# alibaba/euler

Measured on NVIDIA H100. Metric: sampled_edges_per_sec, higher is better.
Workload: dtype u64 ids / f32 weights+features (f64 CDF compare)

## Files before the change

### euler_b200/_lib.py

```python
import ctypes as C
import os

_HERE = os.path.dirname(os.path.abspath(__file__))
SO_PATH = os.path.join(_HERE, "lib", "libeuler_b200.so")

EU_RNG_MINSTD = 0
EU_RNG_PHILOX = 1


class EulerError(RuntimeError):
    pass


class GraphDesc(C.Structure):
    _fields_ = [
        ("n_nodes", C.c_int64), ("n_edge_types", C.c_int32), ("n_node_types", C.c_int32),
        ("ids", C.c_void_p), ("node_type", C.c_void_p), ("node_w", C.c_void_p),
        ("grp_ptr", C.c_void_p), ("nbr", C.c_void_p), ("cum_w", C.c_void_p), ("grp_cum", C.c_void_p),
        ("w", C.c_void_p), ("feat_dim", C.c_int32), ("feat", C.c_void_p),
        ("sampler_order", C.c_void_p), ("n_feat_slots", C.c_int32), ("feat_slot_dims", C.c_void_p),
        ("n_u64_slots", C.c_int32), ("u64_ptr", C.c_void_p), ("u64_val", C.c_void_p),
        ("n_bin_slots", C.c_int32), ("bin_ptr", C.c_void_p), ("bin_val", C.c_void_p),
    ]

# ... 69 lines not shown
    "eu_graph_feat_dim": (_I32, [_P]),
    "eu_graph_hbm_bytes": (_I64, [_P]),
    "eu_graph_export": (C.c_int, [_P] * 9),
    "eu_graph_edge_type_id": (_I32, [_P, C.c_char_p]),
    "eu_graph_node_type_id": (_I32, [_P, C.c_char_p]),
    "eu_graph_dense_feature_id": (_I32, [_P, C.c_char_p]),
    "eu_graph_dense_feature_dim": (_I32, [_P, _I32]),
    "eu_graph_sparse_feature_id": (_I32, [_P, C.c_char_p]),
    "eu_graph_binary_feature_id": (_I32, [_P, C.c_char_p]),
    "eu_get_sparse_feature": (C.c_int, [_P, _P, _I64, _I32, _I64, _I64, _P, _P]),
    "eu_get_sparse_feature_host": (C.c_int, [_P, _P, _I64, _I32, _I64, _I64, _P, _P, _P]),
    "eu_get_binary_feature": (C.c_int, [_P, _P, _I64, _I32, _I64, _P, _P]),
    "eu_get_binary_feature_host": (C.c_int, [_P, _P, _I64, _I32, _I64, _P, _P, _P]),
    "eu_ctx_create": (C.c_int, [_P, C.c_int, _U64, _P, C.POINTER(_P)]),
    "eu_ctx_destroy": (C.c_int, [_P]),
    "eu_ctx_set_stream": (C.c_int, [_P, _P]),
    "eu_ctx_seed": (C.c_int, [_P, _U64]),
    "eu_ctx_set_engines": (C.c_int, [_P, _I32, _P]),
    "eu_ctx_reserve": (C.c_int, [_P, _I64]),
    "eu_ctx_sync": (C.c_int, [_P]),
    "eu_ctx_draws": (C.c_int, [_P, C.POINTER(_U64)]),
    "eu_ctx_profile": (C.c_int, [_P, C.c_int]),
    "eu_ctx_profile_read": (C.c_int, [_P, C.c_char_p, _I64]),
    "eu_sample_neighbor": (C.c_int, [_P, _P, _I64, _P, _I32, _I32, _I64, _P, _P, _P]),
    "eu_sample_neighbor_host": (C.c_int, [_P, _P, _I64, _P, _I32, _I32, _I64, _P, _P, _P]),
    "eu_sample_neighbor_raw": (C.c_int, [_P, _P, _I64, _P, _I32, _I32, _P, _P, _P]),
    "eu_sample_neighbor_raw_host": (C.c_int, [_P, _P, _I64, _P, _I32, _I32, _P, _P, _P]),
    "eu_get_sorted_full_neighbor": (C.c_int, [_P, _P, _I64, _P, _I32, _I64, _P, _P, _P, _P]),
    "eu_get_top_k_neighbor": (C.c_int, [_P, _P, _I64, _P, _I32, _I32, _I64, _P, _P, _P]),
    "eu_sample_neighbor_layerwise": (C.c_int, [_P, _P, _I64, _I32, _P, _I32, _I32, _I64, _I32, _P, _P]),
    "eu_sparse_get_adj": (C.c_int, [_P, _P, _P, _I64, _I32, _I32, _P, _I32, _P]),
    "eu_sparse_get_adj_coo": (C.c_int, [_P, _P, _P, _I64, _I32, _I32, _P, _I32, _I64, _P, _P, _P]),
    "eu_gen_pair_count": (_I64, [_I32, _I32, _I32]),
    "eu_gen_pair": (C.c_int, [_P, _P, _I64, _I32, _I32, _I32, _P]),
    "eu_sample_fanout": (C.c_int, [_P, _P, _I64, _P, _I32, _P, _I32, _I64, _P, _P, _P]),
    "eu_sample_fanout_batched": (C.c_int, [_P, _P, _I32, _I64, _P, _I32, _P, _I32, _I64, _P, _P, _P]),
    "eu_sample_fanout_host": (C.c_int, [_P, _P, _I64, _P, _I32, _P, _I32, _I64, _P, _P, _P]),
    "eu_sample_fanout_batched_host": (C.c_int, [_P, _P, _I32, _I64, _P, _I32, _P, _I32, _I64, _P, _P, _P]),
    "eu_sample_fanout_with_feature": (C.c_int, [_P, _P, _I64, _P, _I32, _P, _I32, _I64, _P, _P, _P, _P, _I32, _P, _P, _P, _I32, _P, _P,
                                                _P, _P]),
    "eu_sage_mean_aggregate_host": (C.c_int, [_P, _P, _I64, _I32, _I32, _P]),
    "eu_sample_node": (C.c_int, [_P, _I32, _P, _I32, _P]),
    "eu_sample_node_host": (C.c_int, [_P, _I32, _P, _I32, _P]),
    "eu_build_alias_table": (C.c_int, [_P, _I64, _P, _P, _P]),
    "eu_graph_load_inspect": (C.c_int, [C.c_char_p, C.c_int, C.c_int, _P, _P, _P, _P, _I64, _P, _P]),
    "eu_random_walk": (C.c_int, [_P, _P, _I64, _P, _I32, _I32, _F, _F, _I64, _P]),
# ... 97 lines not shown
```

### euler_b200/csrc/capi.cu

```cuda
#include <stdio.h>
#include <stdlib.h>
#include <string.h>

#include <algorithm>
#include <map>
#include <mutex>
#include <string>

#include "internal.h"

namespace eu {

__global__ void k_seed(EuRngState* rs, int n, unsigned long long seed0, const unsigned long long* seeds) {
  const int e = blockIdx.x * blockDim.x + threadIdx.x;
  if (e >= n) return;
  const unsigned long long seed = seeds ? seeds[e] : seed0 + (unsigned long long)e;
  EuRngState* r = rs + e;
  unsigned long long x = seed % 2147483647ull;
  r->x = x == 0 ? 1u : (uint32_t)x;
  r->x_prev = r->x;
  r->draws = 0;
  r->calls = 0;
  r->blocks_done = 0;
  r->key = seed * 0x9E3779B97F4A7C15ull;
// ... 25 lines not shown
  int rc;
  if ((table_slots > c->tab_set_slots || rows > c->cap_rows) && (rc = refuse_growth_in_capture(c, "the sampling scratch"))) return rc;
  if (table_slots > c->tab_set_slots) {
    EU_CUDA(cudaStreamSynchronize(c->stream));
    const int64_t slots = table_slots + 64;
    if ((rc = regrow(&c->d_dedup, 2 * slots))) return rc;
    c->tab_set_slots = slots;
    for (int64_t off = 0; off < 2 * slots; off += (int64_t)1 << 20) {
      int64_t n = std::min<int64_t>((int64_t)1 << 20, 2 * slots - off);
      EU_CUDA(cudaMemset2DAsync(&c->d_dedup[off].key, sizeof(HashSlot), 0x00, 8, (size_t)n, c->stream));
      EU_CUDA(cudaMemset2DAsync(&c->d_dedup[off].row, sizeof(HashSlot), 0xFF, 8, (size_t)n, c->stream));
    }
  }
  if (rows <= c->cap_rows) return EU_OK;
  EU_CUDA(cudaStreamSynchronize(c->stream));
  if ((rc = regrow(&c->d_first, rows))) return rc;
  if ((rc = regrow(&c->d_rowof, rows))) return rc;
  if ((rc = regrow(&c->d_elig, rows))) return rc;
  if ((rc = regrow(&c->d_state, rows))) return rc;
  if ((rc = regrow(&c->d_emask, rows / 32 + 2))) return rc;
  if ((rc = regrow(&c->d_woff, rows / 32 + 2))) return rc;
  if ((rc = regrow(&c->d_blkpre, rows / 256 + 66))) return rc;
  if ((rc = regrow(&c->d_blkmul, rows / 256 + 66))) return rc;
  if ((rc = regrow(&c->d_live, rows))) return rc;
  if ((rc = regrow(&c->d_dup, rows))) return rc;
  if (!c->d_nlive && (rc = regrow(&c->d_nlive, 4))) return rc;
  if ((rc = regrow(&c->d_front[0], rows))) return rc;
  if ((rc = regrow(&c->d_front[1], rows))) return rc;
  c->cap_rows = rows;
  return EU_OK;
}

int ctx_misc(eu_ctx* c, int64_t bytes) {
  if (bytes <= c->misc_bytes) return EU_OK;
  if (int rc0 = refuse_growth_in_capture(c, "the op scratch")) return rc0;
  EU_CUDA(cudaStreamSynchronize(c->stream));
  char* p = (char*)c->d_misc;
  int rc = regrow(&p, bytes);
  c->d_misc = p;
  if (rc) { c->misc_bytes = 0; return rc; }
  c->misc_bytes = bytes;
  return EU_OK;
}

int agg_reserve(eu_ctx* c, int64_t rows, int64_t table_slots) {
  if (rows <= c->agg_rows && table_slots <= c->agg_slots) return EU_OK;
  int rc;
// ... 201 lines not shown
```

### euler_b200/csrc/internal.h

```cpp
#pragma once
#include <cuda_runtime.h>
#include <stdint.h>

#include <atomic>
#include <string>
#include <vector>

#include "../../include/euler_b200.h"
#include "common.cuh"

namespace eu {

void set_error(const char* fmt, ...);
extern std::atomic<uint64_t> g_launches;

#define EU_CUDA(call)                                                                    \
  do {                                                                                   \
    cudaError_t _e = (call);                                                             \
    if (_e != cudaSuccess) {                                                             \
      ::eu::set_error("%s:%d %s -> %s", __FILE__, __LINE__, #call, cudaGetErrorString(_e)); \
      return EU_ERR_CUDA;                                                                \
    }                                                                                    \
  } while (0)

// ... 80 lines not shown
};

struct eu_ctx {
  eu_graph* g = nullptr;
  eu_rng_kind rng = EU_RNG_MINSTD;
  uint64_t seed = 0;
  cudaStream_t stream = nullptr;
  EuRngState* d_rng = nullptr;
  int n_eng = 1;
  int64_t cap_rows = 0;
  eu::HashSlot* d_dedup = nullptr;
  int64_t tab_set_slots = 0;
  int32_t* d_first = nullptr;
  int64_t* d_rowof = nullptr;
  uint8_t* d_elig = nullptr;
  uint32_t* d_state = nullptr;
  uint32_t* d_emask = nullptr;
  uint32_t* d_woff = nullptr;
  uint32_t* d_blkpre = nullptr;
  uint32_t* d_blkmul = nullptr;
  int32_t* d_live = nullptr;
  int32_t* d_dup = nullptr;
  unsigned int* d_nlive = nullptr;
  unsigned long long* d_front[2] = {nullptr, nullptr};
  int64_t agg_rows = 0, agg_slots = 0;
  unsigned long long* d_agg_tab = nullptr;
  int32_t* d_agg_src = nullptr;
  int32_t* d_agg_rep = nullptr;
  uint32_t* d_agg_slot = nullptr;
  unsigned int* d_agg_nrep = nullptr;
  void* d_misc = nullptr;
  int64_t misc_bytes = 0;
  float* d_walkv = nullptr;
  long long walkv_cap = 0;
  cudaStream_t aux[2] = {nullptr, nullptr};
  cudaEvent_t ev_fork = nullptr, ev_join[2] = {nullptr, nullptr};
  void* h_pin = nullptr;
  int64_t pin_bytes = 0;
  void* d_stage = nullptr;
  int64_t stage_bytes = 0;
  bool prof = false;
  struct ProfRec { const char* name; int64_t rows; cudaEvent_t e0, e1; };
  std::vector<ProfRec> prof_recs;
};

struct EuProfScope {
// ... 43 lines not shown
```

### euler_b200/csrc/sample.cu

```cuda
#include <algorithm>

#include <stdlib.h>

#include "internal.h"

namespace eu {

struct ETypes {
  int32_t K;
  int32_t v[EU_MAX_ETYPES];
};

struct Geom {
  int32_t nb;
  int32_t nblk_b;
  int64_t rows_b;
  int64_t rows_pad;
  int64_t cap_b;
  const int32_t* rows_act;
};

__global__ void k_dedup_insert(HashSlot* tabs, Geom gm, const unsigned long long* __restrict__ seeds) {
  const int b = blockIdx.y;
  const int64_t li = blockIdx.x * (int64_t)blockDim.x + threadIdx.x;
// ... 35 lines not shown
  if (mode == 1) {
    float s = 0.f;
    for (int32_t i = 0; i < et.K; ++i) {
      int32_t t = et.v[i];
      if (t < 0 || t >= T) return false;
      float pre = t > 0 ? grp_cum_at(g, row, t - 1) : 0.f;
      s = __fadd_rn(s, __fsub_rn(grp_cum_at(g, row, t), pre));
    }
    return s != 0.f;
  }
  return grp_cum_at(g, row, T - 1) != 0.f;
}

struct PrepOut {
  unsigned long long* eng_ids;
  long long* out_ids;
  float* out_w;
  int32_t* out_t;
  int32_t count;
  long long default_node;
  HashSlot* next_tabs;
  int64_t next_cap_b;
  int32_t* live;
  unsigned int* n_live;
  int32_t* dup;
  unsigned int* n_dup;
};

static constexpr int kPrepBlock = 256;

__global__ void __launch_bounds__(kPrepBlock) k_prepare(DevGraph g, const HashSlot* tabs, Geom gm,
                                                        const unsigned long long* __restrict__ seeds,
                                                        ETypes et, int mode, uint32_t F, unsigned long long draws_per_row,
                                                        int32_t* first, int64_t* rowof, uint32_t* emask, uint32_t* wmul,
                                                        uint32_t* blkpre, uint32_t* blkmul, EuRngState* rngs, PrepOut po) {
  __shared__ uint32_t s_w[kPrepBlock / 32];
  __shared__ uint32_t s_l[kPrepBlock / 32];
  __shared__ uint32_t s_d[kPrepBlock / 32];
  __shared__ uint32_t s_z[kPrepBlock / 32];
  __shared__ bool s_last;
  const int b = blockIdx.y;
  const int64_t li = blockIdx.x * (int64_t)kPrepBlock + threadIdx.x;
  const int64_t ii = b * gm.rows_pad + li;
  const int lane = threadIdx.x & 31, wid = threadIdx.x >> 5;
  EuRngState* rng = rngs + b;
  bool e = false;
  bool own = false;
  bool dflt = false;
  const int64_t rows_here = gm.rows_act ? (int64_t)gm.rows_act[b] : gm.rows_b;
  const uint32_t nblk_act = (uint32_t)max((int64_t)1, (rows_here + kPrepBlock - 1) / kPrepBlock);
  if (blockIdx.x >= nblk_act) return;
  if (li < rows_here) {
    const int64_t w = b * gm.rows_b + li;
    const unsigned long long id = seeds[w];
    const int64_t f = tabs ? dedup_first(tabs + (int64_t)b * (gm.cap_b + 1), (unsigned long long)dedup_cap_eff(gm.cap_b, gm.rows_act, b) - 1, id) : li;
    first[ii] = (int32_t)f;
    const int64_t row = lookup_row(g, id);
    own = row_eligible(g, row, et, mode);
    e = own && f == li;
    dflt = !own;
    if (own) rowof[ii] = row;
  }
  const uint32_t zm = __ballot_sync(0xffffffffu, dflt);
  if (zm) {
    const int64_t ob = (b * gm.rows_b + (li - lane)) * (int64_t)po.count;
    const uint32_t n = 32u * (uint32_t)po.count;
    for (uint32_t k = lane; k < n; k += 32) {
      if (!((zm >> (k / (uint32_t)po.count)) & 1u)) continue;
      if (po.eng_ids) po.eng_ids[ob + k] = 0ull;
      if (po.out_ids) { po.out_ids[ob + k] = po.default_node; po.out_w[ob + k] = 0.f; po.out_t[ob + k] = -1; }
    }
  }
  const uint32_t m = __ballot_sync(0xffffffffu, e);
  const uint32_t lm = po.dup ? m : __ballot_sync(0xffffffffu, own);
  const uint32_t dm = po.dup ? __ballot_sync(0xffffffffu, own && !e) : 0u;
  if (lane == 0) { s_w[wid] = __popc(m); s_l[wid] = __popc(lm); s_d[wid] = __popc(dm); s_z[wid] = zm; }
  __syncthreads();
  if (lane == 0) {
    uint32_t off = 0;
    for (int k = 0; k < wid; ++k) off += s_w[k];
    emask[ii >> 5] = m;
    uint32_t fp = 1, fb = F;
    for (; off; off >>= 1) { if (off & 1) fp = modmul(fp, fb); fb = modmul(fb, fb); }
    wmul[ii >> 5] = fp;
  }
  uint32_t* bp = blkpre + (int64_t)b * gm.nblk_b;
  if (threadIdx.x == 0) {
    uint32_t tot = 0, lt = 0, dt = 0;
    for (int k = 0; k < kPrepBlock / 32; ++k) {
      tot += s_w[k];
      const uint32_t l = s_l[k], d = s_d[k];
      s_l[k] = lt; s_d[k] = dt;
      lt += l; dt += d;
    }
    const uint32_t lbase = lt ? atomicAdd(po.n_live, lt) : 0u, dbase = dt ? atomicAdd(po.n_dup, dt) : 0u;
    for (int k = 0; k < kPrepBlock / 32; ++k) { s_l[k] += lbase; s_d[k] += dbase; }
    if (po.next_tabs)
      for (int k = 0; k < kPrepBlock / 32; ++k)
        if (s_z[k]) {
          const int64_t lz = blockIdx.x * (int64_t)kPrepBlock + k * 32 + (__ffs(s_z[k]) - 1);
          dedup_insert_one(po.next_tabs + (int64_t)b * (po.next_cap_b + 1), (unsigned long long)po.next_cap_b - 1, 0ull,
                           lz * (int64_t)po.count);
          break;
        }
    bp[blockIdx.x] = tot;
    __threadfence();
    s_last = atomicAdd(&rng->blocks_done, 1u) == nblk_act - 1;
  }
  __syncthreads();
  {
    const uint32_t below = (1u << lane) - 1u;
    if (e || (own && !po.dup)) po.live[s_l[wid] + __popc(lm & below)] = (int32_t)(b * gm.rows_b + li);
    else if (own) po.dup[s_d[wid] + __popc(dm & below)] = (int32_t)(b * gm.rows_b + li);
  }
  if (!s_last) return;
  __threadfence();
  __shared__ uint32_t s_scan[kPrepBlock];
  uint32_t carry = 0;
  for (uint32_t base = 0; base < nblk_act; base += kPrepBlock) {
    const uint32_t k = base + threadIdx.x;
    const uint32_t v = k < nblk_act ? __ldcg(bp + k) : 0u;
    s_scan[threadIdx.x] = v;
    __syncthreads();
    for (int off = 1; off < kPrepBlock; off <<= 1) {
      uint32_t t = threadIdx.x >= off ? s_scan[threadIdx.x - off] : 0u;
      __syncthreads();
      s_scan[threadIdx.x] += t;
      __syncthreads();
    }
    if (k < nblk_act) {
      uint32_t pre = carry + s_scan[threadIdx.x] - v;
      bp[k] = pre;
      uint32_t fp = 1, fb = F;
      for (; pre; pre >>= 1) { if (pre & 1) fp = modmul(fp, fb); fb = modmul(fb, fb); }
      blkmul[(int64_t)b * gm.nblk_b + k] = fp;
    }
// ... 32 lines not shown
    __syncthreads();
  }
  const uint32_t x0 = rng->x;
  uint32_t run = modmul(x0, t > 0 ? s_part[t - 1] : 1u);
  for (int64_t i = b; i < e; ++i) {
    state[i] = run;
    if (elig[i]) run = modmul(run, F);
  }
  __syncthreads();
  if (t == 1023) {
    rng->x = modmul(x0, s_part[1023]);
    rng->draws += (unsigned long long)s_cnt[1023] * draws_per_row;
  }
}

struct SampleArgs {
  const unsigned long long* seeds;
  Geom gm;
  int32_t count;
  long long default_node;
  ETypes et;
  int mode;
  const int32_t* live;
  const unsigned int* n_live;
  const int32_t* first;
  const int64_t* rowof;
  const uint32_t* emask;
  const uint32_t* wmul;
  const uint32_t* blkmul;
  uint32_t F;
  uint32_t lanepow[32];
  uint32_t stride;
  int sg_log;
  int stage;
  HashSlot* clear_tab;
  int64_t clear_n;
  HashSlot* next_tabs;
  int64_t next_cap_b;
  unsigned long long key;
  const EuRngState* rngs;
  unsigned long long* eng_ids;
  long long* out_ids;
  float* out_w;
  int32_t* out_t;
};

__device__ __forceinline__ int lane_upper_bound(float c, int lo, int hi, float thr, unsigned gmask, int SG) {
#pragma unroll
  for (int it = 0; it < 5; ++it) {
    int mid = (lo + hi) >> 1;
    float v = __shfl_sync(gmask, c, mid, SG);
    bool go = lo < hi;
    bool gt = v >= thr;
    hi = (go && gt) ? mid : hi;
    lo = (go && !gt) ? mid + 1 : lo;
  }
  return lo;
}

__device__ __forceinline__ int32_t bisect_clamped(const float* __restrict__ base, int32_t lo, int32_t hi, float thr) {
  while (lo < hi) {
    const int32_t mid = (lo + hi) >> 1;
    if (__ldg(base + mid) >= thr) hi = mid; else lo = mid + 1;
  }
  return lo;
}

template <bool PHILOX, int CTAS>
__global__ void __launch_bounds__(256, CTAS) k_sample(DevGraph g, SampleArgs a) {
  const int lane = threadIdx.x & 31;
  const int64_t gtid = blockIdx.x * (int64_t)blockDim.x + threadIdx.x;
  __shared__ uint32_t s_lanepow[32];
  __shared__ uint32_t s_fpow[32];
  constexpr int kStageF = 16;
  __shared__ __align__(128) float s_stage[256 * kStageF];
  __shared__ __align__(8) unsigned long long s_bar[32];
  const int SG = 1 << a.sg_log;
  const int sl = lane & (SG - 1);
  const unsigned gmask = SG == 32 ? 0xffffffffu : (((1u << SG) - 1u) << (lane - sl));
  const bool can_stage = a.sg_log >= 3 && a.stage;
  unsigned long long* const bar = &s_bar[can_stage ? (threadIdx.x >> a.sg_log) : 0];
  float* const sm = s_stage + (threadIdx.x - sl) * kStageF;
  const int64_t capg = (int64_t)SG * kStageF;
  uint32_t phase = 0;
  if (can_stage && sl == 0) mbar_init(bar, 1);
  if (!PHILOX && threadIdx.x < 32) {
    s_lanepow[threadIdx.x] = a.lanepow[threadIdx.x];
    uint32_t fp = 1, fb = a.F;
    for (uint32_t e = threadIdx.x; e; e >>= 1) { if (e & 1) fp = modmul(fp, fb); fb = modmul(fb, fb); }
    s_fpow[threadIdx.x] = fp;
  }
  fence_mbar_init();
  __syncthreads();
  if (!PHILOX) {
    if (!a.gm.rows_act) {
      for (int64_t s = gtid; s < a.clear_n; s += (int64_t)gridDim.x * blockDim.x) { a.clear_tab[s].key = 0; a.clear_tab[s].row = kEmptyRow; }
    } else if (a.clear_n) {
      for (int b = 0; b < a.gm.nb; ++b) {
        HashSlot* tab = a.clear_tab + (int64_t)b * (a.gm.cap_b + 1);
        const int64_t n = dedup_cap_eff(a.gm.cap_b, a.gm.rows_act, b) + 1;
        for (int64_t s = gtid; s < n; s += (int64_t)gridDim.x * blockDim.x) { tab[s].key = 0; tab[s].row = kEmptyRow; }
      }
    }
  }
  const int32_t count = a.count;
  const int32_t T = g.T;
  const int64_t total = PHILOX ? a.gm.nb * a.gm.rows_b : (int64_t)__ldg(a.n_live);
  const int64_t qstride = (((int64_t)gridDim.x * blockDim.x) >> 5) << (5 - a.sg_log);
  const uint32_t upd = a.mode == 0 ? 1u : 2u;
  const uint32_t stride = a.stride;

  for (int64_t q = ((gtid >> 5) << (5 - a.sg_log)) + (lane >> a.sg_log); q < total; q += qstride) {
    const int64_t w = PHILOX ? q : (int64_t)a.live[q];
    const int bidx = (int)(w / a.gm.rows_b);
    const int64_t li = w - bidx * a.gm.rows_b;
    if (PHILOX && a.gm.rows_act && li >= a.gm.rows_act[bidx]) continue;
    const int64_t obase = w * (int64_t)count;
    const EuRngState* rng = a.rngs + bidx;
    HashSlot* ntab = a.next_tabs ? a.next_tabs + (int64_t)bidx * (a.next_cap_b + 1) : nullptr;
    const unsigned long long nmask = (unsigned long long)a.next_cap_b - 1;
    const int64_t nbase = li * (int64_t)count;

    int64_t row;
    bool ok;
    uint32_t st = 0;
    unsigned long long seed_id = 0;
    if (PHILOX) {
      seed_id = a.seeds[w];
      row = lookup_row(g, seed_id);
      ok = row_eligible(g, row, a.et, a.mode);
    } else {
      const int64_t ib = bidx * a.gm.rows_pad;
      const int32_t f = a.first[ib + li];
      const uint32_t m = a.emask[(ib + f) >> 5];
      ok = (m >> (f & 31)) & 1u;
      if (ok) {
        row = a.rowof[ib + li];
        st = modmul(modmul(rng->x_prev, a.blkmul[(int64_t)bidx * a.gm.nblk_b + f / kPrepBlock]),
                    modmul(a.wmul[(ib + f) >> 5], s_fpow[__popc(m & ((1u << (f & 31)) - 1u))]));
      } else {
        row = -1;
      }
    }
    if (!ok) {
      for (int32_t j = sl; j < count; j += SG) {
        if (a.eng_ids) a.eng_ids[obase + j] = 0ull;
        if (a.out_ids) { a.out_ids[obase + j] = a.default_node; a.out_w[obase + j] = 0.f; a.out_t[obase + j] = -1; }
      }
      if (!PHILOX && ntab && sl == 0) dedup_insert_one(ntab, nmask, 0ull, nbase);
      continue;
    }

    const int64_t* gp = g.grp_ptr + row * T;
    const int64_t base = gp[0];
    const int64_t rlen = gp[T] - base;
    const bool small_row = rlen <= SG;
    float c = __int_as_float(0x7f800000);
    if (small_row && sl < rlen) c = __ldg(g.cum_w + base + sl);
    const int mis = (int)((reinterpret_cast<uintptr_t>(g.cum_w + base) & 15u) >> 2);
    const bool mid_row = can_stage && !small_row && rlen + mis <= capg;
    if (mid_row && sl == 0) {
      const uint32_t bytes = (uint32_t)((((rlen + mis) << 2) + 15) & ~15ll);
      fence_proxy_async_smem();
      mbar_arrive_expect_tx(bar, bytes);
      bulk_copy_g2s(sm, g.cum_w + base - mis, bytes, bar);
    }
    const float* const srow = sm + mis;

    int64_t gb = 0, ge = 0;
    float lim_b = 0.f, lim_e = 0.f;
    if (a.mode == 0) {
      const int32_t t = a.et.v[0];
      gb = gp[t];
      ge = gp[t + 1] - 1;
      lim_b = gb == base ? 0.f : __ldg(g.cum_w + gb - 1);
      lim_e = __ldg(g.cum_w + ge);
    }
    float tc = __int_as_float(0x7f800000);
    int ntc = 0;
    if (a.mode == 1) {
      ntc = a.et.K;
      float sum = 0.f, mine = 0.f;
      for (int32_t i = 0; i < ntc; ++i) {
        int32_t t = a.et.v[i];
        float pre = t > 0 ? grp_cum_at(g, row, t - 1) : 0.f;
        sum = __fadd_rn(sum, __fsub_rn(grp_cum_at(g, row, t), pre));
        if (i == sl) mine = sum;
      }
      if (sl < ntc) tc = mine;
    } else if (a.mode == 2) {
      ntc = T;
      if (sl < T) tc = grp_cum_at(g, row, sl);
    }
    const float tc_end = __shfl_sync(gmask, tc, ntc > 0 ? ntc - 1 : 0, SG);

    uint32_t x = 0;
    if (!PHILOX) x = modmul(st, s_lanepow[sl]);
    const uint32_t salt = PHILOX ? (uint32_t)rng->calls : 0u;
    const unsigned long long pkey = PHILOX ? a.key ^ rng->key : 0ull;

    if (mid_row) {
      const long long t0 = clock64();
      while (!mbar_try_wait(bar, phase))
        if (clock64() - t0 > 4000000000LL) __trap();
      phase ^= 1u;
    }
    bool keep = true;
    bool bad = false;
    for (int32_t j0 = 0; j0 < count; j0 += SG) {
      const int32_t j = j0 + sl;
      const bool active = j < count;
      double u_t = 0.0, u_n = 0.0;
      if (PHILOX) {
        philox_uniform2(seed_id, (uint32_t)j, salt, pkey, u_t, u_n);
      } else {
        uint32_t xs = x;
        if (upd == 2u) u_t = minstd_uniform(xs);
        u_n = minstd_uniform(xs);
        x = modmul(x, stride);
      }
      int32_t etype = a.mode == 0 ? a.et.v[0] : 0;
      int64_t b = gb, e = ge;
      float lb = lim_b, le = lim_e;
      if (a.mode != 0) {
        const float tt = gt_threshold(pick_r(u_t, 0.f, tc_end));
        int k = lane_upper_bound(tc, 0, ntc - 1, tt, gmask, SG);
        etype = a.mode == 1 ? a.et.v[k] : k;
        b = gp[etype];
        e = gp[etype + 1] - 1;
        if (e < b) {
          bad = bad || active;
          b = base; e = base;
        }
        lb = b == base ? 0.f : __ldg(g.cum_w + b - 1);
        le = __ldg(g.cum_w + e);
      }
      const float thr = gt_threshold(pick_r(u_n, lb, le));
      int64_t m;
      float wgt;
      if (small_row) {
        int li2 = lane_upper_bound(c, (int)(b - base), (int)(e - base), thr, gmask, SG);
        float hi_v = __shfl_sync(gmask, c, li2, SG);
        float lo_v = __shfl_sync(gmask, c, li2 > 0 ? li2 - 1 : 0, SG);
        m = base + li2;
        wgt = __fsub_rn(hi_v, li2 > 0 ? lo_v : 0.f);
      } else if (mid_row) {
        int lo = (int)(b - base), hi = (int)(e - base);
        while (lo < hi) {
          const int mid = (lo + hi) >> 1;
          if (srow[mid] >= thr) hi = mid; else lo = mid + 1;
        }
        m = base + lo;
        wgt = __fsub_rn(srow[lo], lo > 0 ? srow[lo - 1] : 0.f);
      } else {
        m = b + bisect_clamped(g.cum_w + b, 0, (int32_t)(e - b), thr);
        float hi_v = __ldg(g.cum_w + m);
        float lo_v = m > base ? __ldg(g.cum_w + m - 1) : 0.f;
        wgt = __fsub_rn(hi_v, lo_v);
      }
      const unsigned long long nid = active ? __ldg(g.nbr + m) : 0ull;
      if (j0 == 0) {
        unsigned long long first_id = __shfl_sync(gmask, nid, 0, SG);
        keep = first_id != 0ull;
      }
      if (active) {
        if (a.eng_ids) a.eng_ids[obase + j] = nid;
        if (a.out_ids) {
          a.out_ids[obase + j] = keep ? (long long)nid : a.default_node;
          a.out_w[obase + j] = keep ? wgt : 0.f;
          a.out_t[obase + j] = keep ? etype : -1;
        }
      }
      if (!PHILOX && ntab && a.mode == 0) {
        const unsigned act = __ballot_sync(gmask, active);
        if (active) {
          const unsigned peers = __match_any_sync(act, nid);
          if (lane == __ffs(peers) - 1) dedup_insert_one(ntab, nmask, nid, nbase + j);
        }
      }
    }
    if (__any_sync(gmask, bad)) {
      for (int32_t j = sl; j < count; j += SG) {
        if (a.eng_ids) a.eng_ids[obase + j] = 0ull;
        if (a.out_ids) { a.out_ids[obase + j] = a.default_node; a.out_w[obase + j] = 0.f; a.out_t[obase + j] = -1; }
      }
    }
    if (!PHILOX && ntab && a.mode != 0) {
      for (int32_t j0 = 0; j0 < count; j0 += SG) {
        const int32_t j = j0 + sl;
        const bool active = j < count;
        const unsigned long long nid = active ? a.eng_ids[obase + j] : 0ull;
        const unsigned act = __ballot_sync(gmask, active);
        if (active) {
          const unsigned peers = __match_any_sync(act, nid);
          if (lane == __ffs(peers) - 1) dedup_insert_one(ntab, nmask, nid, nbase + j);
        }
      }
    }
    if (mid_row) __syncwarp(gmask);
  }
}

__global__ void __launch_bounds__(256) k_copy_dups(Geom gm, int32_t count, int sg_log, const int32_t* __restrict__ dup,
                                                   const unsigned int* __restrict__ n_dup, const int32_t* __restrict__ first,
                                                   unsigned long long* eng_ids, long long* out_ids, float* out_w, int32_t* out_t) {
  const int sl = threadIdx.x & ((1 << sg_log) - 1);
  const int64_t total = (int64_t)__ldg(n_dup);
  const int64_t stride = ((int64_t)gridDim.x * blockDim.x) >> sg_log;
  for (int64_t q = (blockIdx.x * (int64_t)blockDim.x + threadIdx.x) >> sg_log; q < total; q += stride) {
    const int64_t w = __ldg(dup + q);
    const int bidx = (int)(w / gm.rows_b);
    const int64_t li = w - bidx * gm.rows_b;
    const int64_t f = __ldg(first + bidx * gm.rows_pad + li);
    const int64_t src = (bidx * gm.rows_b + f) * count, dst = w * (int64_t)count;
    for (int32_t j = sl; j < count; j += 1 << sg_log) {
      if (eng_ids) eng_ids[dst + j] = eng_ids[src + j];
      if (out_ids) { out_ids[dst + j] = out_ids[src + j]; out_w[dst + j] = out_w[src + j]; out_t[dst + j] = out_t[src + j]; }
    }
  }
}

__global__ void k_bump_calls(EuRngState* rngs, int nb) {
// ... 112 lines not shown
  int rc = classify(d, etypes, K, &a.et, &a.mode);
  if (rc) return rc;
  if (a.mode != 0 && d.T > 32) { set_error("T > 32 unsupported"); return EU_ERR_UNSUPPORTED; }
  cudaStream_t s = c->stream;
  Geom gm = make_geom(nb, rows_b);
  gm.rows_act = rows_act;
  a.seeds = seeds; a.gm = gm; a.count = count; a.default_node = default_node;
  a.eng_ids = eng_ids; a.out_ids = (long long*)out_ids; a.out_w = out_w; a.out_t = out_t;
  a.rngs = c->d_rng;
  {
    int need = std::min<int>(count, 32);
    if (a.mode == 1) need = std::max<int>(need, std::min<int>(a.et.K, 32));
    if (a.mode == 2) need = std::max<int>(need, std::min<int>(d.T, 32));
    a.sg_log = 0;
    while ((1 << a.sg_log) < need) ++a.sg_log;
  }
  static const int stage_rows = [] { const char* e = getenv("EU_SAMPLE_STAGE"); return e ? (atoi(e) != 0 ? 1 : 0) : 1; }();
  a.stage = stage_rows;
  static const int grid_ctas = [] { const char* e = getenv("EU_SAMPLE_CTAS"); return e ? std::min(8, std::max(1, atoi(e))) : 8; }();
  const int ctas = grid_ctas <= 5 ? 5 : grid_ctas == 6 ? 6 : 8;
  const unsigned blocks = (unsigned)std::min<int64_t>(ceil_div(ceil_div(rows * 32, (int64_t)(32 >> a.sg_log)), 256), kSMs * grid_ctas);
  if (c->rng == EU_RNG_PHILOX) {
    a.key = c->seed;
    { EuProfScope ps(c, "k_sample<philox>", rows); if (ctas == 6) k_sample<true, 6><<<blocks, 256, 0, s>>>(d, a); else k_sample<true, 8><<<blocks, 256, 0, s>>>(d, a); }
    EU_LAUNCHED();
    k_bump_calls<<<1, 64, 0, s>>>(c->d_rng, nb);
    EU_LAUNCHED();
    return EU_OK;
  }
  if (rows >= ((int64_t)1 << 31) || nb > 64) { set_error("rows >= 2^31 or more than 64 batches"); return EU_ERR_UNSUPPORTED; }
  const Geom ng = make_geom(nb, rows_b * count);
  const bool chain = insert_next && eng_ids;
  rc = ctx_reserve(c, std::max(gm.rows_pad, chain ? ng.rows_pad : 0) * nb, (std::max(gm.cap_b, chain ? ng.cap_b : 0) + 1) * nb);
  if (rc) return rc;
  const int tb = kPrepBlock;
  HashSlot* tabs = c->d_dedup + (hop_index & 1) * c->tab_set_slots;
  HashSlot* ntabs = c->d_dedup + ((hop_index + 1) & 1) * c->tab_set_slots;
  if (raw && (pre_inserted || insert_next)) { set_error("hop: raw mode does not chain"); return EU_ERR_INVALID; }
  if (!pre_inserted && !raw) {
    EuProfScope ps(c, "k_dedup_insert", rows);
    k_dedup_insert<<<dim3((unsigned)ceil_div(gm.rows_b, tb), (unsigned)nb), tb, 0, s>>>(tabs, gm, seeds);
    EU_LAUNCHED();
  }
  const unsigned long long upr = (unsigned long long)count * (a.mode == 0 ? 1 : 2);
  const uint32_t F = modpow_a(2ull * upr);
  { EuProfScope ps(c, "k_prepare", rows);
    PrepOut po{};
    po.eng_ids = eng_ids; po.out_ids = (long long*)out_ids; po.out_w = out_w; po.out_t = out_t;
    po.count = count; po.default_node = default_node;
    if (chain) { po.next_tabs = ntabs; po.next_cap_b = ng.cap_b; }
    po.live = c->d_live; po.n_live = c->d_nlive;
    if (!raw && rows >= kRepeatMinRows) { po.dup = c->d_dup; po.n_dup = c->d_nlive + 1; }
    EU_CUDA(cudaMemsetAsync(c->d_nlive, 0, 2 * sizeof(unsigned int), s));
    k_prepare<<<dim3((unsigned)gm.nblk_b, (unsigned)nb), tb, 0, s>>>(d, raw ? nullptr : tabs, gm, seeds, a.et, a.mode, F, upr, c->d_first,
                                                                     c->d_rowof, c->d_emask, c->d_woff, c->d_blkpre, c->d_blkmul,
                                                                     c->d_rng, po); }
  EU_LAUNCHED();
  a.first = c->d_first; a.rowof = c->d_rowof; a.emask = c->d_emask; a.wmul = c->d_woff; a.blkmul = c->d_blkmul;
  a.live = c->d_live; a.n_live = c->d_nlive;
  a.F = F;
  const uint32_t upd = a.mode == 0 ? 1u : 2u;
  for (uint32_t k = 0; k < 32; ++k) a.lanepow[k] = modpow_a(2ull * upd * k);
  a.stride = modpow_a(2ull * upd * (unsigned long long)(1u << a.sg_log));
  a.clear_tab = tabs;
  a.clear_n = raw ? 0 : (gm.cap_b + 1) * nb;
  if (chain) {
    a.next_tabs = ntabs;
    a.next_cap_b = ng.cap_b;
  }
  { EuProfScope ps(c, "k_sample<minstd>", rows);
    if (ctas == 5) k_sample<false, 5><<<blocks, 256, 0, s>>>(d, a);
    else if (ctas == 6) k_sample<false, 6><<<blocks, 256, 0, s>>>(d, a);
    else k_sample<false, 8><<<blocks, 256, 0, s>>>(d, a); }
  EU_LAUNCHED();
  if (!raw && rows >= kRepeatMinRows) {
    EuProfScope ps(c, "k_copy_dups", rows);
    k_copy_dups<<<blocks, 256, 0, s>>>(gm, count, a.sg_log, c->d_dup, c->d_nlive + 1, c->d_first, eng_ids, (long long*)out_ids, out_w, out_t);
    EU_LAUNCHED();
  }
  return EU_OK;
}

}

using namespace eu;

extern "C" {

int eu_sample_neighbor(eu_ctx* c, const int64_t* nodes, int64_t B, const int32_t* etypes, int32_t K,
                       int32_t count, int64_t default_node, int64_t* out_ids, float* out_w,
                       int32_t* out_t) {
  if (!c || B < 0 || count < 0 || (K > 0 && !etypes)) { set_error("eu_sample_neighbor: bad argument"); return EU_ERR_INVALID; }
  EU_CUDA(cudaSetDevice(c->g->device));
  return hop(c, (const unsigned long long*)nodes, B, etypes, K, count, default_node, nullptr, out_ids, out_w, out_t, 0, false, false, 1);
}

int eu_sample_neighbor_raw(eu_ctx* c, const int64_t* nodes, int64_t B, const int32_t* etypes, int32_t K,
                           int32_t count, int64_t* out_ids, float* out_w, int32_t* out_t) {
  if (!c || B < 0 || count < 0 || (K > 0 && !etypes)) { set_error("eu_sample_neighbor_raw: bad argument"); return EU_ERR_INVALID; }
  EU_CUDA(cudaSetDevice(c->g->device));
// ... 79 lines not shown
    }
  }
  char* m = (char*)c->d_misc;
  if (n_sparse > 0) EU_CUDA(cudaMemsetAsync(m, 0, 16 * (size_t)NS, c->stream));
  for (int l = 0; l <= L; ++l) {
    const int64_t* ids = l == 0 ? nodes : eng_ids[l - 1];
    for (int j = 0; j < n_dense; ++j)
      if ((rc = eu_get_dense_feature(c, ids, rows[l], dense_fids[j], dense_dims[j], out_dense[l * n_dense + j]))) return rc;
    for (int j = 0; j < n_sparse; ++j) {
      const int k = l * n_sparse + j;
      if ((rc = sparse_entry_ptr(c, ids, rows[l], sparse_fids[j], m + o_tmp, tmp, sparse_ptr[k]))) return rc;
      k_ragged_stats<<<(unsigned)std::min<int64_t>(ceil_div(rows[l] + 1, 256), kSMs * 8), 256, 0, c->stream>>>((const long long*)sparse_ptr[k], rows[l], (long long*)m + 2 * k);
      EU_LAUNCHED();
    }
  }
  if (n_sparse == 0) return EU_OK;
  std::vector<int64_t> st(2 * (size_t)NS);
  EU_CUDA(cudaMemcpyAsync(st.data(), m, 16 * (size_t)NS, cudaMemcpyDeviceToHost, c->stream));
  EU_CUDA(cudaStreamSynchronize(c->stream));
  for (int k = 0; k < NS; ++k) { sparse_total[k] = st[2 * k]; sparse_max_len[k] = st[2 * k + 1]; }
  return EU_OK;
}

int eu_sample_node(eu_ctx* c, int32_t count, const int32_t* types, int32_t n_types, int64_t* out) {
  if (!c || count < 0 || n_types < 1 || !types) { set_error("eu_sample_node: bad argument"); return EU_ERR_INVALID; }
  eu_graph* g = c->g;
  EU_CUDA(cudaSetDevice(g->device));
  int rc = graph_build_sampler(g);
  if (rc) return rc;
  const int32_t NT = g->d.n_node_types;
  if (NT > EU_MAX_ETYPES) { set_error("more than %d node types", EU_MAX_ETYPES); return EU_ERR_UNSUPPORTED; }
  NodeSamplerDev s{};
  s.n_types = NT;
  for (int t = 0; t < NT; ++t) {
    s.ids[t] = g->samplers[t].ids; s.prob[t] = g->samplers[t].prob; s.alias[t] = g->samplers[t].alias;
    s.n[t] = g->samplers[t].n;
  }
  s.type_prob = g->d_type_prob; s.type_alias = g->d_type_alias;
  uint32_t upd;
  if (n_types == 1) {
    int32_t t = types[0];
    if (t == -1) {
      if (g->type_fwc_sum == 0.f) { set_error("sample_node: total node weight is 0"); return EU_ERR_STATE; }
      s.mode = 1; upd = 4;
    } else {
      if (t < 0 || t >= NT) { set_error("sample_node: node type %d out of range", t); return EU_ERR_INVALID; }
// ... 27 lines not shown
```

### include/euler_b200.h

```cpp
#ifndef EULER_B200_H_
#define EULER_B200_H_

#include <stdbool.h>
#include <stdint.h>

#ifdef __cplusplus
extern "C" {
#endif

typedef enum {
  EU_OK = 0,
  EU_ERR_INVALID = 1,
  EU_ERR_CUDA = 2,
  EU_ERR_NO_GPU = 3,
  EU_ERR_UNSUPPORTED = 4,
  EU_ERR_IO = 5,
  EU_ERR_STATE = 6
} eu_status;

typedef enum { EU_RNG_MINSTD = 0, EU_RNG_PHILOX = 1 } eu_rng_kind;

typedef struct eu_graph eu_graph;
typedef struct eu_ctx eu_ctx;

// ... 69 lines not shown
int eu_build_alias_table(const float* weights, int64_t n, float* prob, int32_t* alias, float* sum);
int32_t eu_graph_num_node_types(const eu_graph* g);
int32_t eu_graph_feat_dim(const eu_graph* g);
int64_t eu_graph_hbm_bytes(const eu_graph* g);
int eu_graph_export(const eu_graph* g, uint64_t* ids, int32_t* node_type, float* node_w,
                    int64_t* grp_ptr, uint64_t* nbr, float* cum_w, float* grp_cum, float* feat);
int32_t eu_graph_edge_type_id(const eu_graph* g, const char* name);
int32_t eu_graph_node_type_id(const eu_graph* g, const char* name);
int32_t eu_graph_dense_feature_id(const eu_graph* g, const char* name);
int32_t eu_graph_dense_feature_dim(const eu_graph* g, int32_t fid);
int32_t eu_graph_sparse_feature_id(const eu_graph* g, const char* name);
int32_t eu_graph_binary_feature_id(const eu_graph* g, const char* name);

int eu_ctx_create(eu_graph* g, eu_rng_kind rng, uint64_t seed, void* stream, eu_ctx** out);
int eu_ctx_destroy(eu_ctx* c);
int eu_ctx_set_stream(eu_ctx* c, void* stream);
int eu_ctx_seed(eu_ctx* c, uint64_t seed);
int eu_ctx_set_engines(eu_ctx* c, int32_t n, const uint64_t* seeds);
int eu_ctx_reserve(eu_ctx* c, int64_t max_rows);
int eu_ctx_sync(eu_ctx* c);
int eu_ctx_draws(eu_ctx* c, uint64_t* draws);
int eu_ctx_profile(eu_ctx* c, int enable);
int eu_ctx_profile_read(eu_ctx* c, char* buf, int64_t cap);

int eu_sample_neighbor(eu_ctx* c, const int64_t* nodes, int64_t B, const int32_t* etypes, int32_t K,
                       int32_t count, int64_t default_node, int64_t* out_ids, float* out_w,
                       int32_t* out_t);
int eu_sample_neighbor_host(eu_ctx* c, const int64_t* nodes, int64_t B, const int32_t* etypes,
                            int32_t K, int32_t count, int64_t default_node, int64_t* out_ids,
                            float* out_w, int32_t* out_t);
int eu_sample_neighbor_raw(eu_ctx* c, const int64_t* nodes, int64_t B, const int32_t* etypes, int32_t K,
                           int32_t count, int64_t* out_ids, float* out_w, int32_t* out_t);
int eu_sample_neighbor_raw_host(eu_ctx* c, const int64_t* nodes, int64_t B, const int32_t* etypes, int32_t K,
                                int32_t count, int64_t* out_ids, float* out_w, int32_t* out_t);
int eu_sample_fanout(eu_ctx* c, const int64_t* nodes, int64_t B, const int32_t* etypes, int32_t K,
                     const int32_t* counts, int32_t L, int64_t default_node, int64_t* const* out_ids,
                     float* const* out_w, int32_t* const* out_t);
int eu_sample_fanout_batched(eu_ctx* c, const int64_t* nodes, int32_t nb, int64_t B, const int32_t* etypes, int32_t K,
                             const int32_t* counts, int32_t L, int64_t default_node, int64_t* const* out_ids,
                             float* const* out_w, int32_t* const* out_t);
int eu_sample_fanout_host(eu_ctx* c, const int64_t* nodes, int64_t B, const int32_t* etypes,
                          int32_t K, const int32_t* counts, int32_t L, int64_t default_node,
                          int64_t* const* out_ids, float* const* out_w, int32_t* const* out_t);
int eu_sample_fanout_batched_host(eu_ctx* c, const int64_t* nodes, int32_t nb, int64_t B, const int32_t* etypes,
                                  int32_t K, const int32_t* counts, int32_t L, int64_t default_node,
                                  int64_t* const* out_ids, float* const* out_w, int32_t* const* out_t);
// ... 242 lines not shown
```

Measured before the change: 6.016 billion.

## Bin live rows by size class in prepare and sample each class separately

The prepare kernel now classifies each live row as small, staged (fits in shared memory) or hub and writes it to one of three per-class compacted lists with separate counters. The sample kernel walks hubs first, then staged, then small rows, so the class is known at compile time and warps see uniform control flow and less divergence. Rows that fail the eligibility check are no longer special-cased in the minstd path. A mode-0 template specialization and a debug API for reading the class lists are also added. The cost is three times the live-list memory, extra ballots and atomics in prepare, and three passes of grid-stride loops.

Result: faster. 6.116 billion, median of 6 (+1.7%).

```diff
diff --git a/euler_b200/_lib.py b/euler_b200/_lib.py
--- a/euler_b200/_lib.py
+++ b/euler_b200/_lib.py
@@ -115,6 +115,7 @@
     "eu_ctx_draws": (C.c_int, [_P, C.POINTER(_U64)]),
     "eu_ctx_profile": (C.c_int, [_P, C.c_int]),
     "eu_ctx_profile_read": (C.c_int, [_P, C.c_char_p, _I64]),
+    "eu_ctx_row_class_list": (C.c_int, [_P, _I32, _P, _I64, _P]),
     "eu_sample_neighbor": (C.c_int, [_P, _P, _I64, _P, _I32, _I32, _I64, _P, _P, _P]),
     "eu_sample_neighbor_host": (C.c_int, [_P, _P, _I64, _P, _I32, _I32, _I64, _P, _P, _P]),
     "eu_sample_neighbor_raw": (C.c_int, [_P, _P, _I64, _P, _I32, _I32, _P, _P, _P]),
diff --git a/euler_b200/csrc/capi.cu b/euler_b200/csrc/capi.cu
--- a/euler_b200/csrc/capi.cu
+++ b/euler_b200/csrc/capi.cu
@@ -71,7 +71,7 @@
   if ((rc = regrow(&c->d_woff, rows / 32 + 2))) return rc;
   if ((rc = regrow(&c->d_blkpre, rows / 256 + 66))) return rc;
   if ((rc = regrow(&c->d_blkmul, rows / 256 + 66))) return rc;
-  if ((rc = regrow(&c->d_live, rows))) return rc;
+  if ((rc = regrow(&c->d_live, 3 * rows))) return rc;
   if ((rc = regrow(&c->d_dup, rows))) return rc;
   if (!c->d_nlive && (rc = regrow(&c->d_nlive, 4))) return rc;
   if ((rc = regrow(&c->d_front[0], rows))) return rc;
diff --git a/euler_b200/csrc/internal.h b/euler_b200/csrc/internal.h
--- a/euler_b200/csrc/internal.h
+++ b/euler_b200/csrc/internal.h
@@ -126,6 +126,7 @@
   int32_t* d_live = nullptr;
   int32_t* d_dup = nullptr;
   unsigned int* d_nlive = nullptr;
+  int64_t live_stride = 0;
   unsigned long long* d_front[2] = {nullptr, nullptr};
   int64_t agg_rows = 0, agg_slots = 0;
   unsigned long long* d_agg_tab = nullptr;
diff --git a/euler_b200/csrc/sample.cu b/euler_b200/csrc/sample.cu
--- a/euler_b200/csrc/sample.cu
+++ b/euler_b200/csrc/sample.cu
@@ -1,4 +1,5 @@
 #include <algorithm>
+#include <type_traits>
 
 #include <stdlib.h>
 
@@ -81,10 +82,27 @@
   HashSlot* next_tabs;
   int64_t next_cap_b;
   int32_t* live;
+  int64_t live_stride;
   unsigned int* n_live;
   int32_t* dup;
   unsigned int* n_dup;
+  int sg_log;
+  int stage;
 };
+
+enum RowClass { kRowSmall = 0, kRowStaged = 1, kRowHub = 2, kRowAny = 3 };
+static constexpr int kStageF = 16;
+
+__host__ __device__ __forceinline__ bool stage_ok(int sg_log, int stage) { return sg_log >= 3 && stage; }
+
+__device__ __forceinline__ int stage_mis(const DevGraph& g, int64_t base) {
+  return (int)((reinterpret_cast<uintptr_t>(g.cum_w + base) & 15u) >> 2);
+}
+
+__device__ __forceinline__ int row_class(const DevGraph& g, int64_t base, int64_t rlen, int sg_log, bool can_stage) {
+  if (rlen <= (1 << sg_log)) return kRowSmall;
+  return can_stage && rlen + stage_mis(g, base) <= ((int64_t)kStageF << sg_log) ? kRowStaged : kRowHub;
+}
 
 static constexpr int kPrepBlock = 256;
 
@@ -94,7 +112,7 @@
                                                         int32_t* first, int64_t* rowof, uint32_t* emask, uint32_t* wmul,
                                                         uint32_t* blkpre, uint32_t* blkmul, EuRngState* rngs, PrepOut po) {
   __shared__ uint32_t s_w[kPrepBlock / 32];
-  __shared__ uint32_t s_l[kPrepBlock / 32];
+  __shared__ uint32_t s_l[3][kPrepBlock / 32];
   __shared__ uint32_t s_d[kPrepBlock / 32];
   __shared__ uint32_t s_z[kPrepBlock / 32];
   __shared__ bool s_last;
@@ -106,6 +124,7 @@
   bool e = false;
   bool own = false;
   bool dflt = false;
+  int cls = -1;
   const int64_t rows_here = gm.rows_act ? (int64_t)gm.rows_act[b] : gm.rows_b;
   const uint32_t nblk_act = (uint32_t)max((int64_t)1, (rows_here + kPrepBlock - 1) / kPrepBlock);
   if (blockIdx.x >= nblk_act) return;
@@ -119,6 +138,10 @@
     e = own && f == li;
     dflt = !own;
     if (own) rowof[ii] = row;
+    if (e || (own && !po.dup)) {
+      const int64_t* gp = g.grp_ptr + row * g.T;
+      cls = row_class(g, gp[0], gp[g.T] - gp[0], po.sg_log, stage_ok(po.sg_log, po.stage));
+    }
   }
   const uint32_t zm = __ballot_sync(0xffffffffu, dflt);
   if (zm) {
@@ -131,9 +154,14 @@
     }
   }
   const uint32_t m = __ballot_sync(0xffffffffu, e);
-  const uint32_t lm = po.dup ? m : __ballot_sync(0xffffffffu, own);
+  const uint32_t lm0 = __ballot_sync(0xffffffffu, cls == kRowSmall);
+  const uint32_t lm1 = __ballot_sync(0xffffffffu, cls == kRowStaged);
+  const uint32_t lm2 = __ballot_sync(0xffffffffu, cls == kRowHub);
   const uint32_t dm = po.dup ? __ballot_sync(0xffffffffu, own && !e) : 0u;
-  if (lane == 0) { s_w[wid] = __popc(m); s_l[wid] = __popc(lm); s_d[wid] = __popc(dm); s_z[wid] = zm; }
+  if (lane == 0) {
+    s_w[wid] = __popc(m); s_d[wid] = __popc(dm); s_z[wid] = zm;
+    s_l[0][wid] = __popc(lm0); s_l[1][wid] = __popc(lm1); s_l[2][wid] = __popc(lm2);
+  }
   __syncthreads();
   if (lane == 0) {
     uint32_t off = 0;
@@ -145,15 +173,20 @@
   }
   uint32_t* bp = blkpre + (int64_t)b * gm.nblk_b;
   if (threadIdx.x == 0) {
-    uint32_t tot = 0, lt = 0, dt = 0;
+    uint32_t tot = 0, lt[3] = {0, 0, 0}, dt = 0;
     for (int k = 0; k < kPrepBlock / 32; ++k) {
       tot += s_w[k];
-      const uint32_t l = s_l[k], d = s_d[k];
-      s_l[k] = lt; s_d[k] = dt;
-      lt += l; dt += d;
-    }
-    const uint32_t lbase = lt ? atomicAdd(po.n_live, lt) : 0u, dbase = dt ? atomicAdd(po.n_dup, dt) : 0u;
-    for (int k = 0; k < kPrepBlock / 32; ++k) { s_l[k] += lbase; s_d[k] += dbase; }
+      const uint32_t d = s_d[k];
+      s_d[k] = dt;
+      dt += d;
+      for (int c = 0; c < 3; ++c) { const uint32_t l = s_l[c][k]; s_l[c][k] = lt[c]; lt[c] += l; }
+    }
+    const uint32_t dbase = dt ? atomicAdd(po.n_dup, dt) : 0u;
+    for (int k = 0; k < kPrepBlock / 32; ++k) s_d[k] += dbase;
+    for (int c = 0; c < 3; ++c) {
+      const uint32_t lbase = lt[c] ? atomicAdd(po.n_live + c, lt[c]) : 0u;
+      for (int k = 0; k < kPrepBlock / 32; ++k) s_l[c][k] += lbase;
+    }
     if (po.next_tabs)
       for (int k = 0; k < kPrepBlock / 32; ++k)
         if (s_z[k]) {
@@ -169,8 +202,12 @@
   __syncthreads();
   {
     const uint32_t below = (1u << lane) - 1u;
-    if (e || (own && !po.dup)) po.live[s_l[wid] + __popc(lm & below)] = (int32_t)(b * gm.rows_b + li);
-    else if (own) po.dup[s_d[wid] + __popc(dm & below)] = (int32_t)(b * gm.rows_b + li);
+    if (cls >= 0) {
+      const uint32_t lm = cls == kRowSmall ? lm0 : cls == kRowStaged ? lm1 : lm2;
+      po.live[cls * po.live_stride + s_l[cls][wid] + __popc(lm & below)] = (int32_t)(b * gm.rows_b + li);
+    } else if (own) {
+      po.dup[s_d[wid] + __popc(dm & below)] = (int32_t)(b * gm.rows_b + li);
+    }
   }
   if (!s_last) return;
   __threadfence();
@@ -249,6 +286,7 @@
   ETypes et;
   int mode;
   const int32_t* live;
+  int64_t live_stride;
   const unsigned int* n_live;
   const int32_t* first;
   const int64_t* rowof;
@@ -293,22 +331,21 @@
   return lo;
 }
 
-template <bool PHILOX, int CTAS>
+template <bool PHILOX, bool M0, int CTAS>
 __global__ void __launch_bounds__(256, CTAS) k_sample(DevGraph g, SampleArgs a) {
+  const int mode = M0 ? 0 : a.mode;
   const int lane = threadIdx.x & 31;
   const int64_t gtid = blockIdx.x * (int64_t)blockDim.x + threadIdx.x;
   __shared__ uint32_t s_lanepow[32];
   __shared__ uint32_t s_fpow[32];
-  constexpr int kStageF = 16;
   __shared__ __align__(128) float s_stage[256 * kStageF];
   __shared__ __align__(8) unsigned long long s_bar[32];
   const int SG = 1 << a.sg_log;
   const int sl = lane & (SG - 1);
   const unsigned gmask = SG == 32 ? 0xffffffffu : (((1u << SG) - 1u) << (lane - sl));
-  const bool can_stage = a.sg_log >= 3 && a.stage;
+  const bool can_stage = stage_ok(a.sg_log, a.stage);
   unsigned long long* const bar = &s_bar[can_stage ? (threadIdx.x >> a.sg_log) : 0];
   float* const sm = s_stage + (threadIdx.x - sl) * kStageF;
-  const int64_t capg = (int64_t)SG * kStageF;
   uint32_t phase = 0;
   if (can_stage && sl == 0) mbar_init(bar, 1);
   if (!PHILOX && threadIdx.x < 32) {
@@ -332,13 +369,17 @@
   }
   const int32_t count = a.count;
   const int32_t T = g.T;
-  const int64_t total = PHILOX ? a.gm.nb * a.gm.rows_b : (int64_t)__ldg(a.n_live);
-  const int64_t qstride = (((int64_t)gridDim.x * blockDim.x) >> 5) << (5 - a.sg_log);
-  const uint32_t upd = a.mode == 0 ? 1u : 2u;
+  const uint32_t upd = mode == 0 ? 1u : 2u;
   const uint32_t stride = a.stride;
-
-  for (int64_t q = ((gtid >> 5) << (5 - a.sg_log)) + (lane >> a.sg_log); q < total; q += qstride) {
-    const int64_t w = PHILOX ? q : (int64_t)a.live[q];
+  using Q = typename std::conditional<PHILOX, int64_t, int32_t>::type;
+
+  auto rows_of = [&](auto cls_tag) {
+  constexpr int CLS = decltype(cls_tag)::value;
+  const int32_t* const list = PHILOX ? nullptr : a.live + CLS * a.live_stride;
+  const Q total = PHILOX ? (Q)(a.gm.nb * a.gm.rows_b) : (Q)__ldg(a.n_live + CLS);
+  const Q qstride = (Q)((((int64_t)gridDim.x * blockDim.x) >> 5) << (5 - a.sg_log));
+  for (Q q = (Q)(((gtid >> 5) << (5 - a.sg_log)) + (lane >> a.sg_log)); q < total; q += qstride) {
+    const int64_t w = PHILOX ? q : (int64_t)list[q];
     const int bidx = (int)(w / a.gm.rows_b);
     const int64_t li = w - bidx * a.gm.rows_b;
     if (PHILOX && a.gm.rows_act && li >= a.gm.rows_act[bidx]) continue;
@@ -355,37 +396,33 @@
     if (PHILOX) {
       seed_id = a.seeds[w];
       row = lookup_row(g, seed_id);
-      ok = row_eligible(g, row, a.et, a.mode);
+      ok = row_eligible(g, row, a.et, mode);
     } else {
       const int64_t ib = bidx * a.gm.rows_pad;
       const int32_t f = a.first[ib + li];
       const uint32_t m = a.emask[(ib + f) >> 5];
-      ok = (m >> (f & 31)) & 1u;
-      if (ok) {
-        row = a.rowof[ib + li];
-        st = modmul(modmul(rng->x_prev, a.blkmul[(int64_t)bidx * a.gm.nblk_b + f / kPrepBlock]),
-                    modmul(a.wmul[(ib + f) >> 5], s_fpow[__popc(m & ((1u << (f & 31)) - 1u))]));
-      } else {
-        row = -1;
-      }
-    }
-    if (!ok) {
+      ok = true;
+      row = a.rowof[ib + li];
+      st = modmul(modmul(rng->x_prev, a.blkmul[(int64_t)bidx * a.gm.nblk_b + f / kPrepBlock]),
+                  modmul(a.wmul[(ib + f) >> 5], s_fpow[__popc(m & ((1u << (f & 31)) - 1u))]));
+    }
+    if (PHILOX && !ok) {
       for (int32_t j = sl; j < count; j += SG) {
         if (a.eng_ids) a.eng_ids[obase + j] = 0ull;
         if (a.out_ids) { a.out_ids[obase + j] = a.default_node; a.out_w[obase + j] = 0.f; a.out_t[obase + j] = -1; }
       }
-      if (!PHILOX && ntab && sl == 0) dedup_insert_one(ntab, nmask, 0ull, nbase);
       continue;
     }
 
     const int64_t* gp = g.grp_ptr + row * T;
     const int64_t base = gp[0];
     const int64_t rlen = gp[T] - base;
-    const bool small_row = rlen <= SG;
+    const int cls = CLS == kRowAny ? row_class(g, base, rlen, a.sg_log, can_stage) : CLS;
+    const bool small_row = cls == kRowSmall;
     float c = __int_as_float(0x7f800000);
     if (small_row && sl < rlen) c = __ldg(g.cum_w + base + sl);
-    const int mis = (int)((reinterpret_cast<uintptr_t>(g.cum_w + base) & 15u) >> 2);
-    const bool mid_row = can_stage && !small_row && rlen + mis <= capg;
+    const bool mid_row = cls == kRowStaged;
+    const int mis = mid_row ? stage_mis(g, base) : 0;
     if (mid_row && sl == 0) {
       const uint32_t bytes = (uint32_t)((((rlen + mis) << 2) + 15) & ~15ll);
       fence_proxy_async_smem();
@@ -396,7 +433,7 @@
 
     int64_t gb = 0, ge = 0;
     float lim_b = 0.f, lim_e = 0.f;
-    if (a.mode == 0) {
+    if (mode == 0) {
       const int32_t t = a.et.v[0];
       gb = gp[t];
       ge = gp[t + 1] - 1;
@@ -405,7 +442,7 @@
     }
     float tc = __int_as_float(0x7f800000);
     int ntc = 0;
-    if (a.mode == 1) {
+    if (mode == 1) {
       ntc = a.et.K;
       float sum = 0.f, mine = 0.f;
       for (int32_t i = 0; i < ntc; ++i) {
@@ -415,7 +452,7 @@
         if (i == sl) mine = sum;
       }
       if (sl < ntc) tc = mine;
-    } else if (a.mode == 2) {
+    } else if (mode == 2) {
       ntc = T;
       if (sl < T) tc = grp_cum_at(g, row, sl);
     }
@@ -446,13 +483,13 @@
         u_n = minstd_uniform(xs);
         x = modmul(x, stride);
       }
-      int32_t etype = a.mode == 0 ? a.et.v[0] : 0;
+      int32_t etype = mode == 0 ? a.et.v[0] : 0;
       int64_t b = gb, e = ge;
       float lb = lim_b, le = lim_e;
-      if (a.mode != 0) {
+      if (mode != 0) {
         const float tt = gt_threshold(pick_r(u_t, 0.f, tc_end));
         int k = lane_upper_bound(tc, 0, ntc - 1, tt, gmask, SG);
-        etype = a.mode == 1 ? a.et.v[k] : k;
+        etype = mode == 1 ? a.et.v[k] : k;
         b = gp[etype];
         e = gp[etype + 1] - 1;
         if (e < b) {
@@ -498,7 +535,7 @@
           a.out_t[obase + j] = keep ? etype : -1;
         }
       }
-      if (!PHILOX && ntab && a.mode == 0) {
+      if (!PHILOX && ntab && mode == 0) {
         const unsigned act = __ballot_sync(gmask, active);
         if (active) {
           const unsigned peers = __match_any_sync(act, nid);
@@ -512,7 +549,7 @@
         if (a.out_ids) { a.out_ids[obase + j] = a.default_node; a.out_w[obase + j] = 0.f; a.out_t[obase + j] = -1; }
       }
     }
-    if (!PHILOX && ntab && a.mode != 0) {
+    if (!PHILOX && ntab && mode != 0) {
       for (int32_t j0 = 0; j0 < count; j0 += SG) {
         const int32_t j = j0 + sl;
         const bool active = j < count;
@@ -525,6 +562,14 @@
       }
     }
     if (mid_row) __syncwarp(gmask);
+  }
+  };
+  if (PHILOX) {
+    rows_of(std::integral_constant<int, kRowAny>());
+  } else {
+    rows_of(std::integral_constant<int, kRowHub>());
+    if (can_stage) rows_of(std::integral_constant<int, kRowStaged>());
+    rows_of(std::integral_constant<int, kRowSmall>());
   }
 }
 
@@ -683,7 +728,12 @@
   const unsigned blocks = (unsigned)std::min<int64_t>(ceil_div(ceil_div(rows * 32, (int64_t)(32 >> a.sg_log)), 256), kSMs * grid_ctas);
   if (c->rng == EU_RNG_PHILOX) {
     a.key = c->seed;
-    { EuProfScope ps(c, "k_sample<philox>", rows); if (ctas == 6) k_sample<true, 6><<<blocks, 256, 0, s>>>(d, a); else k_sample<true, 8><<<blocks, 256, 0, s>>>(d, a); }
+    { EuProfScope ps(c, "k_sample<philox>", rows);
+      if (a.mode == 0) {
+        if (ctas == 6) k_sample<true, true, 6><<<blocks, 256, 0, s>>>(d, a); else k_sample<true, true, 8><<<blocks, 256, 0, s>>>(d, a);
+      } else {
+        if (ctas == 6) k_sample<true, false, 6><<<blocks, 256, 0, s>>>(d, a); else k_sample<true, false, 8><<<blocks, 256, 0, s>>>(d, a);
+      } }
     EU_LAUNCHED();
     k_bump_calls<<<1, 64, 0, s>>>(c->d_rng, nb);
     EU_LAUNCHED();
@@ -710,15 +760,16 @@
     po.eng_ids = eng_ids; po.out_ids = (long long*)out_ids; po.out_w = out_w; po.out_t = out_t;
     po.count = count; po.default_node = default_node;
     if (chain) { po.next_tabs = ntabs; po.next_cap_b = ng.cap_b; }
-    po.live = c->d_live; po.n_live = c->d_nlive;
-    if (!raw && rows >= kRepeatMinRows) { po.dup = c->d_dup; po.n_dup = c->d_nlive + 1; }
-    EU_CUDA(cudaMemsetAsync(c->d_nlive, 0, 2 * sizeof(unsigned int), s));
+    po.live = c->d_live; po.live_stride = rows; po.n_live = c->d_nlive;
+    c->live_stride = rows;
+    po.sg_log = a.sg_log; po.stage = a.stage;
+    if (!raw && rows >= kRepeatMinRows) { po.dup = c->d_dup; po.n_dup = c->d_nlive + 3; }
+    EU_CUDA(cudaMemsetAsync(c->d_nlive, 0, 4 * sizeof(unsigned int), s));
     k_prepare<<<dim3((unsigned)gm.nblk_b, (unsigned)nb), tb, 0, s>>>(d, raw ? nullptr : tabs, gm, seeds, a.et, a.mode, F, upr, c->d_first,
                                                                      c->d_rowof, c->d_emask, c->d_woff, c->d_blkpre, c->d_blkmul,
                                                                      c->d_rng, po); }
   EU_LAUNCHED();
   a.first = c->d_first; a.rowof = c->d_rowof; a.emask = c->d_emask; a.wmul = c->d_woff; a.blkmul = c->d_blkmul;
-  a.live = c->d_live; a.n_live = c->d_nlive;
   a.F = F;
   const uint32_t upd = a.mode == 0 ? 1u : 2u;
   for (uint32_t k = 0; k < 32; ++k) a.lanepow[k] = modpow_a(2ull * upd * k);
@@ -729,14 +780,21 @@
     a.next_tabs = ntabs;
     a.next_cap_b = ng.cap_b;
   }
+  a.live = c->d_live; a.live_stride = rows; a.n_live = c->d_nlive;
   { EuProfScope ps(c, "k_sample<minstd>", rows);
-    if (ctas == 5) k_sample<false, 5><<<blocks, 256, 0, s>>>(d, a);
-    else if (ctas == 6) k_sample<false, 6><<<blocks, 256, 0, s>>>(d, a);
-    else k_sample<false, 8><<<blocks, 256, 0, s>>>(d, a); }
+    if (a.mode == 0) {
+      if (ctas == 5) k_sample<false, true, 5><<<blocks, 256, 0, s>>>(d, a);
+      else if (ctas == 6) k_sample<false, true, 6><<<blocks, 256, 0, s>>>(d, a);
+      else k_sample<false, true, 8><<<blocks, 256, 0, s>>>(d, a);
+    } else {
+      if (ctas == 5) k_sample<false, false, 5><<<blocks, 256, 0, s>>>(d, a);
+      else if (ctas == 6) k_sample<false, false, 6><<<blocks, 256, 0, s>>>(d, a);
+      else k_sample<false, false, 8><<<blocks, 256, 0, s>>>(d, a);
+    } }
   EU_LAUNCHED();
   if (!raw && rows >= kRepeatMinRows) {
     EuProfScope ps(c, "k_copy_dups", rows);
-    k_copy_dups<<<blocks, 256, 0, s>>>(gm, count, a.sg_log, c->d_dup, c->d_nlive + 1, c->d_first, eng_ids, (long long*)out_ids, out_w, out_t);
+    k_copy_dups<<<blocks, 256, 0, s>>>(gm, count, a.sg_log, c->d_dup, c->d_nlive + 3, c->d_first, eng_ids, (long long*)out_ids, out_w, out_t);
     EU_LAUNCHED();
   }
   return EU_OK;
@@ -862,6 +920,23 @@
   return EU_OK;
 }
 
+int eu_ctx_row_class_list(eu_ctx* c, int32_t cls, int32_t* out, int64_t cap, int64_t* n) {
+  if (!c || cls < kRowSmall || cls > kRowHub || cap < 0 || (cap > 0 && !out) || !n) { set_error("eu_ctx_row_class_list: bad argument"); return EU_ERR_INVALID; }
+  EU_CUDA(cudaSetDevice(c->g->device));
+  *n = 0;
+  if (!c->d_nlive) return EU_OK;
+  unsigned int h = 0;
+  EU_CUDA(cudaMemcpyAsync(&h, c->d_nlive + cls, sizeof(h), cudaMemcpyDeviceToHost, c->stream));
+  EU_CUDA(cudaStreamSynchronize(c->stream));
+  *n = h;
+  const int64_t k = std::min<int64_t>(cap, h);
+  if (k > 0) {
+    EU_CUDA(cudaMemcpyAsync(out, c->d_live + cls * c->live_stride, (size_t)k * sizeof(int32_t), cudaMemcpyDeviceToHost, c->stream));
+    EU_CUDA(cudaStreamSynchronize(c->stream));
+  }
+  return EU_OK;
+}
+
 int eu_sample_node(eu_ctx* c, int32_t count, const int32_t* types, int32_t n_types, int64_t* out) {
   if (!c || count < 0 || n_types < 1 || !types) { set_error("eu_sample_node: bad argument"); return EU_ERR_INVALID; }
   eu_graph* g = c->g;
diff --git a/include/euler_b200.h b/include/euler_b200.h
--- a/include/euler_b200.h
+++ b/include/euler_b200.h
@@ -115,6 +115,7 @@
 int eu_ctx_draws(eu_ctx* c, uint64_t* draws);
 int eu_ctx_profile(eu_ctx* c, int enable);
 int eu_ctx_profile_read(eu_ctx* c, char* buf, int64_t cap);
+int eu_ctx_row_class_list(eu_ctx* c, int32_t cls, int32_t* out, int64_t cap, int64_t* n);
 
 int eu_sample_neighbor(eu_ctx* c, const int64_t* nodes, int64_t B, const int32_t* etypes, int32_t K,
                        int32_t count, int64_t default_node, int64_t* out_ids, float* out_w,
```
